# antekone/libarchive

Measured on AMD Instinct MI355X. Metric: decompressed MiB/s (whole node), lz4 filter, XXH32 verified, bit-exact, higher is better.
Workload: dtype u8; 1 GPU; C2: raw-format + lz4 filter, 16.00 GiB decoded per GPU, 262144 independent 64 KiB blocks per GPU in frames of 16, block+content+header XXH32 verified; compressed_bytes_per_gpu=7527480016, decoded_bytes_per_gpu=17179869184, unique_region_mib=1024, tiles=16, collectives=RCCL (nccl backend), expand_kernel=auto

## Files before the change

include/la_gpu.h:

```cpp
#ifndef LA_GPU_H
#define LA_GPU_H

#include <stddef.h>
#include <stdint.h>

#ifdef __cplusplus
extern "C" {
#endif

#define LA_GPU_ABI_VERSION 3

typedef enum la_rc {
	LA_OK            = 0,
	LA_ERR_NO_DEVICE = -1,
	LA_ERR_HIP       = -2,
	LA_ERR_ARG       = -3,
	LA_ERR_NOMEM     = -4
} la_rc;

typedef struct la_gpu_ctx la_gpu_ctx;

int         la_gpu_abi_version(void);
int         la_gpu_device_count(void);
int         la_gpu_open(int device, la_gpu_ctx **out);
// ... 141 lines not shown
	la_batch_summary   *d_summary;
	uint32_t            options;
	uint32_t            hist_len;
	const void         *d_carry_in;
	void               *d_carry_out;
} la_lz4_batch;
#define LA_XXH_CARRY_BYTES 64u

uint64_t la_gpu_lz4_workspace_bytes(uint32_t n_blocks, uint64_t src_bytes);

int la_gpu_lz4_decode(la_gpu_ctx *ctx, const la_lz4_batch *batch);

int la_gpu_lz4_debug_deps(la_gpu_ctx *ctx, const la_lz4_batch *batch, uint32_t block, uint64_t *seq_out,
    uint32_t *deps_out, uint32_t cap);

typedef struct la_gz_member {
	uint64_t src_off;
	uint32_t src_len;
	uint32_t dst_cap;
	uint64_t dst_off;
} la_gz_member;

typedef struct la_gz_result {
	uint32_t status;
	uint32_t out_len;
	uint32_t consumed;
	uint32_t crc32;
} la_gz_result;

typedef struct la_gz_batch {
// ... 378 lines not shown
```

libarchive_amd/_native.py:

```python
import ctypes as C
import os

import numpy as np

_PKG = os.path.dirname(os.path.abspath(__file__))
GPU_LIB_PATH = os.environ.get("LA_GPU_LIB") or os.path.join(_PKG, "csrc", "libla_gpu.so")
HOST_LIB_PATH = os.path.join(_PKG, "host", "libla_host.so")

LA_OK = 0

LZ4_BLOCK_DTYPE = np.dtype([("src_off", "<u8"), ("src_len", "<u4"), ("dst_cap", "<u4"),
                            ("flags", "<u4"), ("block_sum", "<u4")])
LZ4_FRAME_DTYPE = np.dtype([("desc_off", "<u8"), ("desc_len", "<u4"), ("first_block", "<u4"),
                            ("n_blocks", "<u4"), ("flags", "<u4"), ("content_sum", "<u4"),
                            ("reserved", "<u4")])
HASH_JOB_DTYPE = np.dtype([("off", "<u8"), ("len", "<u4"), ("seed", "<u4")])
SUMMARY_DTYPE = np.dtype([("total_out", "<u8"), ("n_bad_units", "<u4"), ("n_bad_frames", "<u4"),
                          ("first_bad_unit", "<u4"), ("first_bad_frame", "<u4"),
                          ("first_zero_unit", "<u4"), ("reserved", "<u4")])
GZ_MEMBER_DTYPE = np.dtype([("src_off", "<u8"), ("src_len", "<u4"), ("dst_cap", "<u4"), ("dst_off", "<u8")])
GZ_RESULT_DTYPE = np.dtype([("status", "<u4"), ("out_len", "<u4"), ("consumed", "<u4"), ("crc32", "<u4")])
assert LZ4_BLOCK_DTYPE.itemsize == 24 and LZ4_FRAME_DTYPE.itemsize == 32
assert HASH_JOB_DTYPE.itemsize == 16 and SUMMARY_DTYPE.itemsize == 32

# ... 218 lines not shown
        lib.la_gpu_sync.argtypes = [C.c_void_p]
        lib.la_gpu_last_error.argtypes = [C.c_void_p]
        lib.la_gpu_last_error.restype = C.c_char_p
        lib.la_gpu_reserve.argtypes = [C.c_void_p, C.c_uint64]
        lib.la_gpu_timer_start.argtypes = [C.c_void_p]
        lib.la_gpu_timer_stop.argtypes = [C.c_void_p, C.POINTER(C.c_float)]
        lib.la_gpu_profile_enable.argtypes = [C.c_void_p, C.c_int]
        lib.la_gpu_profile_read.argtypes = [C.c_void_p, C.POINTER(C.c_float), C.POINTER(C.c_char_p), C.c_int]
        lib.la_gpu_xxh32_many.argtypes = [C.c_void_p, C.c_void_p, C.c_void_p, C.c_uint32, C.c_void_p]
        lib.la_gpu_crc32_many.argtypes = [C.c_void_p, C.c_void_p, C.c_void_p, C.c_uint32, C.c_void_p]
        lib.la_gpu_lz4_workspace_bytes.argtypes = [C.c_uint32, C.c_uint64]
        lib.la_gpu_lz4_workspace_bytes.restype = C.c_uint64
        lib.la_gpu_lz4_decode.argtypes = [C.c_void_p, C.POINTER(_Lz4BatchC)]
        lib.la_gpu_lz4_debug_deps.argtypes = [C.c_void_p, C.POINTER(_Lz4BatchC), C.c_uint32, C.c_void_p, C.c_void_p,
                                              C.c_uint32]
        lib.la_gpu_lz4_compress.argtypes = [C.c_void_p, C.POINTER(_Lz4cBatchC)]
        lib.la_gpu_gzip_compress.argtypes = [C.c_void_p, C.POINTER(_GzcBatchC)]
        lib.la_gpu_gzip_compress_bound.restype = C.c_uint64
        lib.la_gpu_gzip_compress_bound.argtypes = [C.c_uint64, C.c_uint32]
        lib.la_gpu_gzip_compress_workspace_bytes.restype = C.c_uint64
        lib.la_gpu_gzip_compress_workspace_bytes.argtypes = [C.c_uint64, C.c_uint32]
        lib.la_gpu_lz4_compress_bound.restype = C.c_uint64
        lib.la_gpu_lz4_compress_bound.argtypes = [C.c_uint64, C.c_uint32, C.c_uint32]
        lib.la_gpu_lz4_compress_workspace_bytes.restype = C.c_uint64
        lib.la_gpu_lz4_compress_workspace_bytes.argtypes = [C.c_uint64, C.c_uint32, C.c_uint32]
        lib.la_gpu_gzip_decode.argtypes = [C.c_void_p, C.POINTER(_GzBatchC)]
        lib.la_gpu_zip_compress.argtypes = [C.c_void_p, C.POINTER(_ZipcBatchC)]
        lib.la_gpu_zip_compress_bound.restype = C.c_uint64
        lib.la_gpu_zip_compress_bound.argtypes = [C.c_uint64, C.c_uint32, C.c_uint32, C.c_uint64]
        lib.la_gpu_zip_compress_workspace_bytes.restype = C.c_uint64
# ... 221 lines not shown
        self._check(gpu_lib().la_gpu_xxh32_many(self._h, d_base_ptr, d_jobs_ptr, n, d_out_ptr), "la_gpu_xxh32_many")

    def crc32_many(self, d_base_ptr, d_jobs_ptr, n, d_out_ptr):
        self._check(gpu_lib().la_gpu_crc32_many(self._h, d_base_ptr, d_jobs_ptr, n, d_out_ptr), "la_gpu_crc32_many")

    def lz4_decode(self, batch: _Lz4BatchC):
        self._check(gpu_lib().la_gpu_lz4_decode(self._h, C.byref(batch)), "la_gpu_lz4_decode")

    def lz4_debug_deps(self, batch: _Lz4BatchC, block: int, cap: int = 4096):
        seq, deps = np.zeros(cap, dtype=np.uint64), np.zeros(cap, dtype=np.uint32)
        n = gpu_lib().la_gpu_lz4_debug_deps(self._h, C.byref(batch), block, seq.ctypes.data, deps.ctypes.data, cap)
        if n < 0:
            self._check(n, "la_gpu_lz4_debug_deps")
        return seq[:min(n, cap)], deps[:min(n, cap)]

    def lz4_compress(self, batch: _Lz4cBatchC):
        self._check(gpu_lib().la_gpu_lz4_compress(self._h, C.byref(batch)), "la_gpu_lz4_compress")

    def zstd_compress(self, batch: _ZstdcBatchC):
        self._check(gpu_lib().la_gpu_zstd_compress(self._h, C.byref(batch)), "la_gpu_zstd_compress")

    def bzip2_compress(self, batch: _Bz2cBatchC):
        self._check(gpu_lib().la_gpu_bzip2_compress(self._h, C.byref(batch)), "la_gpu_bzip2_compress")

    def gzip_compress(self, batch: _GzcBatchC):
        self._check(gpu_lib().la_gpu_gzip_compress(self._h, C.byref(batch)), "la_gpu_gzip_compress")

    def zip_compress(self, batch: _ZipcBatchC) -> int:
        rc = gpu_lib().la_gpu_zip_compress(self._h, C.byref(batch))
        if rc != LA_ERR_ARG:
# ... 38 lines not shown
```

libarchive_amd/csrc/la_api.hip:

```cpp
#include "la_dev.h"
#include <stdio.h>
#include <stdlib.h>
#include <string.h>
#include <new>

#define LA_MAX_SLICES 8
#define LA_GZ_LANES_MIN 8192u
#define LA_PROF_MAX_RANGES 64

struct la_gpu_ctx {
	int device;
	hipStream_t own_stream;
	hipStream_t stream;
	hipEvent_t ev0, ev1;
	hipEvent_t mark;
	void *ws;
	uint64_t ws_bytes;
	uint32_t *lz4_deps;
	uint64_t lz4_deps_cap;
	hipStream_t aux_stream;
	hipEvent_t slice_ev[LA_MAX_SLICES + 1];
	int prof_on;
	int prof_n;
	hipEvent_t prof_a[LA_PROF_MAX_RANGES], prof_b[LA_PROF_MAX_RANGES];
	const char *prof_name[LA_PROF_MAX_RANGES];
	char err[256];
};

static void prof_begin(la_gpu_ctx *c) { c->prof_n = 0; }
static int prof_open(la_gpu_ctx *c, const char *name, hipStream_t s)
{
	if (!c->prof_on || c->prof_n >= LA_PROF_MAX_RANGES)
		return -1;
	int h = c->prof_n++;
// ... 65 lines not shown
	for (int i = 0; i <= LA_MAX_SLICES; i++)
		(void)hipEventCreateWithFlags(&c->slice_ev[i], hipEventDisableTiming);
	c->stream = c->own_stream;
	*out = c;
	return LA_OK;
}

void la_gpu_close(la_gpu_ctx *c)
{
	if (!c)
		return;
	(void)hipSetDevice(c->device);
	(void)hipStreamSynchronize(c->stream);
	if (c->ws) (void)hipFree(c->ws);
	if (c->lz4_deps) (void)hipFree(c->lz4_deps);
	(void)hipEventDestroy(c->ev0);
	(void)hipEventDestroy(c->ev1);
	(void)hipEventDestroy(c->mark);
	for (int i = 0; i < LA_PROF_MAX_RANGES; i++) {
		(void)hipEventDestroy(c->prof_a[i]);
		(void)hipEventDestroy(c->prof_b[i]);
	}
	for (int i = 0; i <= LA_MAX_SLICES; i++)
		(void)hipEventDestroy(c->slice_ev[i]);
	(void)hipStreamSynchronize(c->aux_stream);
	(void)hipStreamDestroy(c->aux_stream);
	(void)hipStreamDestroy(c->own_stream);
	delete c;
}

// ... 185 lines not shown

uint64_t la_gpu_lz4_workspace_bytes(uint32_t n_blocks, uint64_t src_bytes)
{
	lz4_ws w;
	lz4_ws_carve(&w, NULL, n_blocks, src_bytes, true);
	return w.total;
}

static int lz4_deps_reserve(la_gpu_ctx *c, uint64_t words)
{
	if (words <= c->lz4_deps_cap)
		return LA_OK;
	HIPCHK(c, hipSetDevice(c->device));
	HIPCHK(c, hipStreamSynchronize(c->stream));
	HIPCHK(c, hipStreamSynchronize(c->aux_stream));
	if (c->lz4_deps) { HIPCHK(c, hipFree(c->lz4_deps)); c->lz4_deps = NULL; c->lz4_deps_cap = 0; }
	words = (words + 0x3FFFFull) & ~0x3FFFFull;
	HIPCHK(c, hipMalloc((void **)&c->lz4_deps, words * sizeof(uint32_t)));
	c->lz4_deps_cap = words;
	return LA_OK;
}

static bool lz4_uses_deps(const la_lz4_batch *bt)
{
	return !(bt->options & (LA_LZ4_OPT_GENERAL_ONLY | LA_LZ4_OPT_SEARCH_IN_EXPAND)) && bt->n_blocks &&
	    ((bt->options & LA_LZ4_OPT_EXPAND_INORDER) == 0 || !la_lz4_expand_inorder_takes(bt->src_bytes));
}

int la_gpu_lz4_decode(la_gpu_ctx *c, const la_lz4_batch *bt)
{
	if (!c || !bt)
		return LA_ERR_ARG;
	if (!bt->d_dst_off || (bt->n_blocks && (!bt->d_src || !bt->d_blocks || !bt->d_dst || !bt->d_out_len ||
// ... 10 lines not shown
		int rc = la_gpu_reserve(c, w.total);
		if (rc != LA_OK) return rc;
	}
	lz4_ws_carve(&w, (uint8_t *)c->ws, bt->n_blocks, bt->src_bytes, fast);
	const bool with_deps = lz4_uses_deps(bt);
	if (with_deps) {
		int rc = lz4_deps_reserve(c, w.table_cap);
		if (rc != LA_OK) return rc;
	}
	hipStream_t sx = c->stream;
	hipStream_t sp = c->aux_stream;
	const uint32_t n = bt->n_blocks;
	const la_expand_job xj = {	 bt->d_src, bt->src_bytes, bt->d_blocks, n, bt->d_dst, bt->dst_cap, bt->d_dst_off,
	    bt->d_out_len, bt->d_block_status, w.nseq, fast ? w.table : NULL, w.table_off,
	    LA_LZ4_LONG_SEQ_BYTES,
	    with_deps ? c->lz4_deps : NULL };

	prof_begin(c);
	HIPCHK(c, hipEventRecord(c->slice_ev[LA_MAX_SLICES], sx));
	HIPCHK(c, hipStreamWaitEvent(sp, c->slice_ev[LA_MAX_SLICES], 0));

	if (n)
		HIPCHK(c, hipMemsetAsync(bt->d_block_status, 0, (size_t)n * sizeof(uint32_t), sp));
	if (fast) {
		la_launch_lz4_table_caps(sp, bt->d_blocks, n, w.caps);
		la_launch_scan_u32(sp, w.caps, n, w.table_off, w.scan);
	}
	if (verify && n)
		HIPCHK(c, hipMemsetAsync(w.sum_status, 0, (size_t)n * sizeof(uint32_t), sp));
	if (bt->options & LA_LZ4_OPT_PARSE_V1) {
		if (verify && n)
// ... 1 lines not shown
		prof_range(c, "lz4_parse", sp, [&] {
			la_launch_lz4_parse(sp, bt->d_src, bt->src_bytes, bt->d_blocks, n, bt->d_out_len, w.nseq,
			    bt->d_block_status, fast ? w.table : NULL, w.table_off, w.table_cap);
		});
	} else {
		prof_range(c, "lz4_parse", sp, [&] {
			la_launch_lz4_parse_staged(sp, bt->d_src, bt->src_bytes, bt->d_blocks, n, bt->d_out_len, w.nseq,
			    bt->d_block_status, verify ? w.sum_status : NULL, fast ? w.table : NULL, w.table_off, w.table_cap);
		});
	}
	HIPCHK(c, hipEventRecord(c->slice_ev[0], sp));

	HIPCHK(c, hipStreamWaitEvent(sx, c->slice_ev[0], 0));
	prof_range(c, "scan", sx, [&] { la_launch_scan_u32(sx, bt->d_out_len, n, bt->d_dst_off, w.scan); });
	if (with_deps)
		prof_range(c, "lz4_deps", sx, [&] { la_launch_lz4_deps(sx, xj, c->lz4_deps); });

	prof_range(c, fast ? "lz4_expand_general" : "lz4_expand", sx, [&] { la_launch_lz4_expand_general(sx, xj, bt->hist_len); });
	if (fast && poll)
		prof_range(c, "lz4_expand_big", sx, [&] { la_launch_lz4_expand_fast_big(sx, xj, w.big); });
	const uint32_t nsl = (fast && n >= 4u * 8192u) ? 4u : 1u;
	if (bt->n_frames && !verify)
		HIPCHK(c, hipMemsetAsync(bt->d_frame_status, 0, (size_t)bt->n_frames * sizeof(uint32_t), sx));
	for (uint32_t i = 0; i < nsl; i++) {
		const uint32_t first = (uint32_t)((uint64_t)n * i / nsl), last = (uint32_t)((uint64_t)n * (i + 1) / nsl);
		const la_expand_job sj = xj.slice(first, last - first);
		if (fast)
			prof_range(c, "lz4_expand", sx, [&] { (poll ? la_launch_lz4_expand_fast : la_launch_lz4_expand_inorder)(sx, sj); });
		if (bt->n_frames && verify) {
			HIPCHK(c, hipEventRecord(c->slice_ev[1 + i], sx));
			HIPCHK(c, hipStreamWaitEvent(sp, c->slice_ev[1 + i], 0));
// ... 31 lines not shown
	HIPCHK(c, hipMemcpyAsync(&ns, w.nseq + block, sizeof(ns), hipMemcpyDeviceToHost, c->stream));
	HIPCHK(c, hipMemcpyAsync(&toff, w.table_off + block, sizeof(toff), hipMemcpyDeviceToHost, c->stream));
	HIPCHK(c, hipStreamSynchronize(c->stream));
	if (ns == 0xFFFFFFFFu)
		return 0;
	if (ns > 0x7FFFFFFFu || toff > w.table_cap || ns > w.table_cap - toff)
		return LA_ERR_ARG;
	const uint32_t m = ns < cap ? ns : cap;
	if (m) {
		static_assert(sizeof(la_lz4_seq) == sizeof(uint64_t), "a table entry travels as one 64-bit value");
		HIPCHK(c, hipMemcpyAsync(seq_out, w.table + toff, (size_t)m * sizeof(uint64_t), hipMemcpyDeviceToHost, c->stream));
		HIPCHK(c, hipMemcpyAsync(deps_out, c->lz4_deps + toff, (size_t)m * sizeof(uint32_t), hipMemcpyDeviceToHost, c->stream));
		HIPCHK(c, hipStreamSynchronize(c->stream));
	}
	return (int)ns;
}

uint64_t la_gpu_zstd_workspace_bytes(uint32_t n_frames)
{
	return la_zstd_workspace_bytes(n_frames);
}

int la_gpu_zstd_decode(la_gpu_ctx *c, const la_zstd_batch *bt)
{
	if (!c || !bt)
		return LA_ERR_ARG;
	if (bt->n_frames && (!bt->d_src || !bt->d_frames || !bt->d_dst || !bt->d_results))
		return LA_ERR_ARG;
	const bool blocks = (bt->options & LA_ZSTD_OPT_BLOCK_PARALLEL) && bt->n_frames && bt->dst_cap <= 0xFFFFFFFFull;
	const uint64_t ws_frames = (la_zstd_workspace_bytes(bt->n_frames) + 255) & ~255ull;
// ... 551 lines not shown
```

libarchive_amd/csrc/la_dev.h:

```cpp
#ifndef LA_DEV_H
#define LA_DEV_H

#include <hip/hip_runtime.h>
#include <stdint.h>
#include "../../include/la_gpu.h"

#define LA_WAVE 64

__device__ __forceinline__ uint32_t ld_u32(const uint8_t *p)
{
	uint32_t v;
	__builtin_memcpy(&v, p, 4);
	return v;
}
__device__ __forceinline__ uint4 ld_u128(const uint8_t *p)
{
	uint4 v;
	__builtin_memcpy(&v, p, 16);
	return v;
}
__device__ __forceinline__ uint32_t rotl32(uint32_t x, int r)
{
	return __builtin_rotateleft32(x, r);
}
// ... 393 lines not shown
	const uint32_t s0 = mdst - off;
	if (mlen == 0 || s0 >= d)
		return false;
	const uint32_t span = mlen < off ? mlen : off;
	uint32_t hi = s0 + span - 1;
	if (hi >= d)
		hi = d - 1;
	*hi_byte = hi;
	return true;
}
__device__ __forceinline__ bool la_lz4_dep_drops_last(uint32_t hi_byte, uint32_t last_mstart)
{
	return hi_byte < last_mstart;
}

struct la_expand_job {
	const uint8_t *src;
	uint64_t src_bytes;
	const la_lz4_block *blocks;
	uint32_t n;
	uint8_t *dst;
	uint64_t dst_cap;
	const uint64_t *dst_off;
	const uint32_t *out_len;
	uint32_t *status;
	const uint32_t *nseq;
	const la_lz4_seq *table;
	const uint64_t *table_off;
	uint32_t long_thr;
	const uint32_t *deps;

	la_expand_job slice(uint32_t first, uint32_t count) const
	{
		return la_expand_job{ src, src_bytes, blocks + first, count, dst, dst_cap, dst_off + first, out_len + first,
		    status + first, nseq + first, table, table_off + first, long_thr, deps };
	}
};

void la_launch_lz4_table_caps(hipStream_t s, const la_lz4_block *d_blocks, uint32_t n, uint32_t *d_caps);
void la_launch_lz4_parse(hipStream_t s, const uint8_t *d_src, uint64_t src_bytes,
    const la_lz4_block *d_blocks, uint32_t n, uint32_t *d_out_len, uint32_t *d_nseq,
    uint32_t *d_status, la_lz4_seq *d_table , const uint64_t *d_table_off,
    uint64_t table_cap );
void la_launch_lz4_parse_staged(hipStream_t s, const uint8_t *d_src, uint64_t src_bytes,
    const la_lz4_block *d_blocks, uint32_t n, uint32_t *d_out_len, uint32_t *d_nseq,
    uint32_t *d_status, uint32_t *d_sum_status, la_lz4_seq *d_table, const uint64_t *d_table_off,
    uint64_t table_cap);
void la_launch_lz4_expand_general(hipStream_t s, const la_expand_job &j, uint32_t hist_len);
void la_launch_lz4_expand_fast(hipStream_t s, const la_expand_job &j);
void la_launch_lz4_expand_fast_big(hipStream_t s, const la_expand_job &j, uint32_t *d_big );
void la_launch_lz4_deps(hipStream_t s, const la_expand_job &j, uint32_t *d_deps);

bool la_lz4_expand_inorder_takes(uint64_t src_bytes);
void la_launch_lz4_expand_inorder(hipStream_t s, const la_expand_job &j);

uint64_t la_zstd_workspace_bytes(uint32_t n_frames);
void la_launch_zstd_frames(hipStream_t s, const uint8_t *d_src, uint64_t src_bytes, const la_zstd_frame *d_frames, uint32_t n,
    uint8_t *d_dst, uint64_t dst_cap, la_zstd_result *d_results, uint8_t *ws, uint32_t options,
    const uint32_t *d_only );
uint64_t la_zstd_blocks_workspace_bytes(uint32_t n_frames, uint64_t src_bytes, uint64_t dst_cap);
const uint32_t *la_zstd_blocks_todo(const uint8_t *ws);
void la_launch_zstd_blocks(hipStream_t s, const uint8_t *d_src, uint64_t src_bytes, const la_zstd_frame *d_frames, uint32_t n,
    uint8_t *d_dst, uint64_t dst_cap, la_zstd_result *d_results, uint8_t *ws, uint32_t options);

uint64_t la_bzip2_workspace_bytes(uint32_t n, uint32_t level);
uint32_t la_bzip2_max_blocks(uint32_t level);
// ... 135 lines not shown
```

libarchive_amd/csrc/la_lz4_deps.hip:

```cpp
#include "la_dev.h"

#define DEPS_THREADS 256
#define DEPS_SLOTS   (LA_LZ4_FAST_MAXSEQ / DEPS_THREADS)

__global__ __launch_bounds__(DEPS_THREADS) void lz4_deps_kernel(const la_lz4_block *__restrict__ blocks, uint32_t n,
    uint64_t dst_cap, const uint64_t *__restrict__ dst_off, const uint32_t *__restrict__ out_len,
    const uint32_t *__restrict__ status, const uint32_t *__restrict__ nseq, const la_lz4_seq *__restrict__ table,
    const uint64_t *__restrict__ table_off, uint32_t long_thr, uint32_t *__restrict__ deps)
{
	__shared__ uint16_t dstpos[LA_LZ4_FAST_MAXSEQ];
	__shared__ uint16_t mstart[LA_LZ4_FAST_MAXSEQ];
	__shared__ uint16_t cmap[2048];

	const uint32_t bi = blockIdx.x;
	if (bi >= n)
		return;
	const uint32_t olen = out_len[bi], ns = nseq[bi];
	if (la_lz4_route(blocks[bi], status[bi], olen, ns, dst_off[bi], dst_cap, true, long_thr) != LA_XR_WINDOW)
		return;
	const uint32_t tid = threadIdx.x;
	const uint64_t *const tab = (const uint64_t *)(const void *)(table + table_off[bi]);
	uint32_t *const out = deps + table_off[bi];

	uint64_t ent[DEPS_SLOTS];
#pragma unroll
	for (uint32_t r = 0; r < DEPS_SLOTS; r++) {
		const uint32_t k = r * DEPS_THREADS + tid;
		ent[r] = k < ns ? tab[k] : 0;
	}
#pragma unroll
	for (uint32_t r = 0; r < DEPS_SLOTS; r++) {
		if (r * DEPS_THREADS >= ns)
			break;
		const uint32_t k = r * DEPS_THREADS + tid;
		if (k < ns) {
			const uint32_t d = (uint32_t)(ent[r] >> 32) & 0xFFFFu;
			dstpos[k] = (uint16_t)d;
			mstart[k] = (uint16_t)(d + ((uint32_t)(ent[r] >> 16) & 0xFFFFu));
		}
	}
	__syncthreads();
#pragma unroll
	for (uint32_t r = 0; r < DEPS_SLOTS; r++) {
		if (r * DEPS_THREADS >= ns)
			break;
		const uint32_t k = r * DEPS_THREADS + tid;
		const uint32_t after = k + 1 < ns ? (uint32_t)dstpos[k + 1] : (olen & 0xFFFFu);
		ent[r] = (ent[r] & ~0xFFFFull) | after;
	}
#pragma unroll
	for (uint32_t r = 0; r < DEPS_SLOTS; r++) {
		if (r * DEPS_THREADS >= ns)
			break;
		const uint32_t k = r * DEPS_THREADS + tid;
		if (k < ns) {
			const uint32_t d = (uint32_t)(ent[r] >> 32) & 0xFFFFu;
			uint32_t nxt = (uint32_t)ent[r] & 0xFFFFu;
			if (nxt < d)
				nxt = 65536u;
			if (k == 0)
				for (uint32_t c = 0; (c << 5) < d; c++)
					cmap[c] = 0;
			for (uint32_t c = (d + 31) >> 5; (c << 5) < nxt; c++)
				cmap[c] = (uint16_t)k;
		}
	}
	__syncthreads();

#pragma unroll
	for (uint32_t r = 0; r < DEPS_SLOTS; r++) {
		if (r * DEPS_THREADS >= ns)
			break;
		const uint32_t k = r * DEPS_THREADS + tid;
		const uint64_t e = ent[r];
// ... 18 lines not shown
		while (q + 1 < kq && dstpos[q + 1] <= s0)
			q++;
		if (qe < q)
			qe = q;
		while (qe + 1 < ke && dstpos[qe + 1] <= hi)
			qe++;
		if (k < ns) {
			uint32_t cnt = 0;
			if (waits)
				cnt = qe - q + 1 - (la_lz4_dep_drops_last(hi, mstart[qe]) ? 1u : 0u);
			out[k] = q | (cnt << 16);
		}
	}
}

void la_launch_lz4_deps(hipStream_t s, const la_expand_job &j, uint32_t *d_deps)
{
	if (j.n == 0) return;
	hipLaunchKernelGGL(lz4_deps_kernel, dim3(j.n), dim3(DEPS_THREADS), 0, s, j.blocks, j.n, j.dst_cap, j.dst_off,
	    j.out_len, j.status, j.nseq, j.table, j.table_off, j.long_thr, d_deps);
}
```

libarchive_amd/csrc/la_lz4_fast.hip:

```cpp
#include "la_dev.h"

#ifndef POLL_SLEEP
#define POLL_SLEEP 1
#endif
#ifndef FAST_THREADS
#define FAST_THREADS 512
#endif
#ifndef LBATCH
#define LBATCH 2
#endif
#ifndef FAST_MIN_WAVES
#define FAST_MIN_WAVES 4
#endif
#define FAST_WAVES   (FAST_THREADS / 64)

#ifdef LA_DIAG
__device__ unsigned long long *la_diag_stamps;
#define STAMP(slot)                                                                       \
	do {                                                                              \
		if (threadIdx.x == 0 && la_diag_stamps)                                    \
			la_diag_stamps[(size_t)blockIdx.x * 8 + (slot)] = __builtin_readcyclecounter(); \
	} while (0)
#else
#define STAMP(slot) do { } while (0)
// ... 15 lines not shown
{
	return *(const uint64_t *)(const void *)(t + k);
}
#define SEQ_LIT_SRC(e) ((uint32_t)((e) & 0xFFFFu))
#define SEQ_LIT_LEN(e) ((uint32_t)(((e) >> 16) & 0xFFFFu))
#define SEQ_DST(e)     ((uint32_t)(((e) >> 32) & 0xFFFFu))
#define SEQ_OFF(e)     ((uint32_t)((e) >> 48))

template <uint32_t MAXSEQ, bool SEG, bool DEPS>
__global__ __launch_bounds__(FAST_THREADS, FAST_MIN_WAVES) void lz4_expand_fast_kernel(
    const uint8_t *__restrict__ src, uint64_t src_bytes, const la_lz4_block *__restrict__ blocks,
    uint32_t n, uint8_t *__restrict__ dst, uint64_t dst_cap, const uint64_t *__restrict__ dst_off,
    const uint32_t *__restrict__ out_len, uint32_t *status_out,
    const uint32_t *__restrict__ nseq, const la_lz4_seq *__restrict__ table,
    const uint64_t *__restrict__ table_off, const uint32_t *__restrict__ big_list,
    const uint32_t *__restrict__ big_count, uint32_t long_thr, const uint32_t *__restrict__ deps)
{
	static_assert(!(SEG && DEPS), "the dependency words number a block's sequences from its first one");
	const uint32_t *status = status_out;
	__shared__ __attribute__((aligned(16))) uint8_t win[16 + 65536 + 96];
	__shared__ uint16_t dstpos[MAXSEQ + 4];
	__shared__ uint32_t donebits[MAXSEQ / 32];
	__shared__ uint16_t chunk_first[2048 + 8];

	auto do_block = [&](const uint32_t bi) __attribute__((always_inline)) {
	if (bi >= n)
		return;
	const la_lz4_block b = blocks[bi];
	const uint32_t olen = out_len[bi];
	const uint32_t ns_all = nseq[bi];
	const uint64_t doff = dst_off[bi];
	static_assert(MAXSEQ == LA_LZ4_FAST_MAXSEQ, "la_lz4_route splits the window kernels' blocks at LA_LZ4_FAST_MAXSEQ");
	if (la_lz4_route(b, status[bi], olen, ns_all, doff, dst_cap, true, long_thr) != (SEG ? LA_XR_WINDOW_SEG : LA_XR_WINDOW))
		return;

	STAMP(0);
	const uint32_t tid = threadIdx.x, lane = tid & 63, wave = tid >> 6;
	const la_lz4_seq *const tab_all = table + table_off[bi];
// ... 10 lines not shown
		vv[u][0] = vv[u][1] = vv[u][2] = vv[u][3] = 0;
		if (c0 < b.src_len) {
			if ((uint64_t)c0 + 32 <= s_room) {
				const uint4 a = ld_u128(s + c0), bq = ld_u128(s + c0 + 16);
				vv[u][0] = ((uint64_t)a.y << 32) | a.x; vv[u][1] = ((uint64_t)a.w << 32) | a.z;
				vv[u][2] = ((uint64_t)bq.y << 32) | bq.x; vv[u][3] = ((uint64_t)bq.w << 32) | bq.z;
			} else {
				for (uint32_t i = 0; c0 + i < s_room && i < 32; i++) {
					const uint64_t by = (uint64_t)s[c0 + i] << (8 * (i & 7));
					if (i < 8) vv[u][0] |= by; else if (i < 16) vv[u][1] |= by;
					else if (i < 24) vv[u][2] |= by; else vv[u][3] |= by;
				}
			}
		}
	}
	auto segment = [&](const uint32_t kb) __attribute__((always_inline)) {
	const la_lz4_seq *const tab = tab_all + kb;
	const uint32_t ns = ns_all - kb < MAXSEQ ? ns_all - kb : MAXSEQ;
	uint32_t cb = 0, seg_prev_end = 0;
	if (kb) {
		const seq_t pvb = seq_load(tab_all, kb - 1);
		seg_prev_end = SEQ_LIT_SRC(pvb) + SEQ_LIT_LEN(pvb);
		cb = seg_prev_end >> 5;
	}
	seq_t ent[MAXSTEPS];
	uint32_t prev_end[MAXSTEPS];
	uint32_t dw[MAXSTEPS];
#pragma unroll
	for (uint32_t r = 0; r < MAXSTEPS; r++) {
		ent[r] = 0;
		prev_end[r] = 0;
		dw[r] = 0;
	}
#pragma unroll
	for (uint32_t r = 0; r < MAXSTEPS; r++) {
		if (r * FAST_THREADS >= ns)
			break;
		const uint32_t k = fast_seq_index(r, wave, lane);
		ent[r] = k < ns ? seq_load(tab, k) : 0;
		const seq_t pv = ((k > 0 || kb > 0) && k < ns) ? seq_load(tab_all, kb + k - 1) : 0;
		prev_end[r] = SEQ_LIT_SRC(pv) + SEQ_LIT_LEN(pv);
	}
	if (tid < MAXSEQ / 32)
		donebits[tid] = 0;
	if (tid == 0) {
		dstpos[ns] = kb + ns < ns_all ? (uint16_t)SEQ_DST(seq_load(tab_all, kb + ns)) : (uint16_t)olen;
		if ((cb << 5) < seg_prev_end)
			chunk_first[0] = 0;
	}
#pragma unroll
	for (uint32_t r = 0; r < MAXSTEPS; r++) {
		if (r * FAST_THREADS >= ns)
			break;
		const uint32_t k = fast_seq_index(r, wave, lane);
		if (k < ns) {
			const uint32_t le = SEQ_LIT_SRC(ent[r]) + SEQ_LIT_LEN(ent[r]);
			for (uint32_t c = (prev_end[r] + 31) >> 5; (c << 5) < le; c++)
				chunk_first[c - cb] = (uint16_t)k;
			dstpos[k] = (uint16_t)SEQ_DST(ent[r]);
			if (k + 1 == ns)
				chunk_first[2048] = (uint16_t)(((le + 31) >> 5) - cb);
		}
	}
	__syncthreads();
#ifdef LA_DIAG_L
	STAMP(6);
#endif

	const uint32_t nlit_chunks = chunk_first[2048];
	for (uint32_t base = 0; base < nlit_chunks; base += LBATCH * FAST_THREADS) {
		uint32_t kk[LBATCH];
		seq_t pe[LBATCH][6];
#pragma unroll
		for (int u = 0; u < LBATCH; u++) {
			const uint32_t c = base + u * FAST_THREADS + tid;
			kk[u] = c < nlit_chunks ? (uint32_t)chunk_first[c] : 0xFFFFFFFFu;
			if (base != 0 || kb != 0) {
				vv[u][0] = vv[u][1] = vv[u][2] = vv[u][3] = 0;
				const uint32_t c0 = (cb + c) << 5;
				if (c < nlit_chunks) {
					if ((uint64_t)c0 + 32 <= s_room) {
						const uint4 a = ld_u128(s + c0), bq = ld_u128(s + c0 + 16);
						vv[u][0] = ((uint64_t)a.y << 32) | a.x; vv[u][1] = ((uint64_t)a.w << 32) | a.z;
						vv[u][2] = ((uint64_t)bq.y << 32) | bq.x; vv[u][3] = ((uint64_t)bq.w << 32) | bq.z;
					} else {
						for (uint32_t i = 0; c0 + i < s_room && i < 32; i++) {
							const uint64_t by = (uint64_t)s[c0 + i] << (8 * (i & 7));
							if (i < 8) vv[u][0] |= by; else if (i < 16) vv[u][1] |= by;
							else if (i < 24) vv[u][2] |= by; else vv[u][3] |= by;
						}
					}
// ... 42 lines not shown
			bool fin = false;
#pragma unroll
			for (int t = 0; t < 6; t++)
				if (!fin)
					fin = (kk[u] + t >= ns) || put(pe[u][t], kb != 0 && kk[u] + t == 0);
			for (uint32_t k = kk[u] + 6; !fin && k < ns; k++)
				fin = put(seq_load(tab, k), false);
		}
	}
	if (DEPS) {
#pragma unroll
		for (uint32_t r = 0; r < MAXSTEPS; r++) {
			const uint32_t k = fast_seq_index(r, wave, lane);
			dw[r] = (r * FAST_THREADS < ns && k < ns) ? deps[table_off[bi] + k] : 0;
		}
	}
	STAMP(1);
	__syncthreads();
	STAMP(2);

	uint32_t qcur[MAXSTEPS];
	if constexpr (DEPS) {
#pragma unroll
		for (uint32_t r = 0; r < MAXSTEPS; r++)
			qcur[r] = dw[r];
#ifdef LA_DIAG_M
		STAMP(6);
#endif
	} else {
#ifndef FAST_BSEARCH
// ... 277 lines not shown
	if (la_lz4_route(blocks[i], status[i], out_len[i], nseq[i], 0, ~0ull, true, long_thr) == LA_XR_WINDOW_SEG)
		big_list[atomicAdd(big_count, 1u)] = i;
}

#ifdef LA_DIAG
extern "C" int la_diag_set_stamps(void *d_buf)
{
	unsigned long long *p = (unsigned long long *)d_buf;
	return (int)hipMemcpyToSymbol(HIP_SYMBOL(la_diag_stamps), &p, sizeof(p));
}
#endif

void la_launch_lz4_expand_fast(hipStream_t s, const la_expand_job &j)
{
	if (j.n == 0) return;
	if (j.deps)
		hipLaunchKernelGGL((lz4_expand_fast_kernel<LA_LZ4_FAST_MAXSEQ, false, true>), dim3(j.n), dim3(FAST_THREADS), 0, s,
		    j.src, j.src_bytes, j.blocks, j.n, j.dst, j.dst_cap, j.dst_off, j.out_len, j.status, j.nseq,
		    j.table, j.table_off, (const uint32_t *)nullptr, (const uint32_t *)nullptr, j.long_thr, j.deps);
	else
		hipLaunchKernelGGL((lz4_expand_fast_kernel<LA_LZ4_FAST_MAXSEQ, false, false>), dim3(j.n), dim3(FAST_THREADS), 0, s,
		    j.src, j.src_bytes, j.blocks, j.n, j.dst, j.dst_cap, j.dst_off, j.out_len, j.status, j.nseq,
		    j.table, j.table_off, (const uint32_t *)nullptr, (const uint32_t *)nullptr, j.long_thr, (const uint32_t *)nullptr);
}

void la_launch_lz4_expand_fast_big(hipStream_t s, const la_expand_job &j, uint32_t *d_big)
{
	if (j.n == 0) return;
	(void)hipMemsetAsync(d_big, 0, sizeof(uint32_t), s);
	hipLaunchKernelGGL(lz4_classify_kernel, dim3((j.n + 255) / 256), dim3(256), 0, s, j.blocks, j.n, j.status, j.nseq,
	    d_big + 1, d_big, j.out_len, j.long_thr);
	const uint32_t grid = j.n < 1024u ? j.n : 1024u;
	hipLaunchKernelGGL((lz4_expand_fast_kernel<LA_LZ4_FAST_MAXSEQ, true, false>), dim3(grid), dim3(FAST_THREADS), 0, s,
	    j.src, j.src_bytes, j.blocks, j.n, j.dst, j.dst_cap, j.dst_off, j.out_len, j.status, j.nseq,
	    j.table, j.table_off, (const uint32_t *)(d_big + 1), (const uint32_t *)d_big, j.long_thr, (const uint32_t *)nullptr);
}
```

Measured before the change: 653,300 MiB/s.

## Precompute literal chunk-to-sequence plan in deps kernel for fast LZ4 expand

The deps kernel now also writes a per-block literal plan that maps each 32-byte literal chunk to the sequence owning it. When deps are present, the fast expand kernel reads this plan from global memory instead of rebuilding chunk_first in shared memory. This removes the prev_end table loads and the shared chunk-map build from the expand kernel and shrinks its shared memory footprint. The cost is an extra device buffer, extra global writes in the deps kernel and extra global reads in expand.

```diff
diff --git a/include/la_gpu.h b/include/la_gpu.h
--- a/include/la_gpu.h
+++ b/include/la_gpu.h
@@ -179,6 +179,9 @@
 int la_gpu_lz4_debug_deps(la_gpu_ctx *ctx, const la_lz4_batch *batch, uint32_t block, uint64_t *seq_out,
     uint32_t *deps_out, uint32_t cap);
 
+int la_gpu_lz4_debug_literal_plan(la_gpu_ctx *ctx, const la_lz4_batch *batch, uint32_t block, uint16_t *plan_out,
+    uint32_t cap);
+
 typedef struct la_gz_member {
 	uint64_t src_off;
 	uint32_t src_len;
diff --git a/libarchive_amd/_native.py b/libarchive_amd/_native.py
--- a/libarchive_amd/_native.py
+++ b/libarchive_amd/_native.py
@@ -256,6 +256,7 @@
         lib.la_gpu_lz4_decode.argtypes = [C.c_void_p, C.POINTER(_Lz4BatchC)]
         lib.la_gpu_lz4_debug_deps.argtypes = [C.c_void_p, C.POINTER(_Lz4BatchC), C.c_uint32, C.c_void_p, C.c_void_p,
                                               C.c_uint32]
+        lib.la_gpu_lz4_debug_literal_plan.argtypes = [C.c_void_p, C.POINTER(_Lz4BatchC), C.c_uint32, C.c_void_p, C.c_uint32]
         lib.la_gpu_lz4_compress.argtypes = [C.c_void_p, C.POINTER(_Lz4cBatchC)]
         lib.la_gpu_gzip_compress.argtypes = [C.c_void_p, C.POINTER(_GzcBatchC)]
         lib.la_gpu_gzip_compress_bound.restype = C.c_uint64
@@ -507,6 +508,13 @@
             self._check(n, "la_gpu_lz4_debug_deps")
         return seq[:min(n, cap)], deps[:min(n, cap)]
 
+    def lz4_debug_literal_plan(self, batch: _Lz4BatchC, block: int, cap: int = 2049):
+        plan = np.zeros(cap, dtype=np.uint16)
+        n = gpu_lib().la_gpu_lz4_debug_literal_plan(self._h, C.byref(batch), block, plan.ctypes.data, cap)
+        if n < 0:
+            self._check(n, "la_gpu_lz4_debug_literal_plan")
+        return plan[:min(n, cap)]
+
     def lz4_compress(self, batch: _Lz4cBatchC):
         self._check(gpu_lib().la_gpu_lz4_compress(self._h, C.byref(batch)), "la_gpu_lz4_compress")
 
diff --git a/libarchive_amd/csrc/la_api.hip b/libarchive_amd/csrc/la_api.hip
--- a/libarchive_amd/csrc/la_api.hip
+++ b/libarchive_amd/csrc/la_api.hip
@@ -18,6 +18,7 @@
 	uint64_t ws_bytes;
 	uint32_t *lz4_deps;
 	uint64_t lz4_deps_cap;
+	uint8_t *lz4_plan;
 	hipStream_t aux_stream;
 	hipEvent_t slice_ev[LA_MAX_SLICES + 1];
 	int prof_on;
@@ -113,6 +114,7 @@
 	(void)hipStreamSynchronize(c->stream);
 	if (c->ws) (void)hipFree(c->ws);
 	if (c->lz4_deps) (void)hipFree(c->lz4_deps);
+	if (c->lz4_plan) (void)hipFree(c->lz4_plan);
 	(void)hipEventDestroy(c->ev0);
 	(void)hipEventDestroy(c->ev1);
 	(void)hipEventDestroy(c->mark);
@@ -328,9 +330,12 @@
 	HIPCHK(c, hipSetDevice(c->device));
 	HIPCHK(c, hipStreamSynchronize(c->stream));
 	HIPCHK(c, hipStreamSynchronize(c->aux_stream));
-	if (c->lz4_deps) { HIPCHK(c, hipFree(c->lz4_deps)); c->lz4_deps = NULL; c->lz4_deps_cap = 0; }
+	c->lz4_deps_cap = 0;
+	if (c->lz4_deps) { HIPCHK(c, hipFree(c->lz4_deps)); c->lz4_deps = NULL; }
+	if (c->lz4_plan) { HIPCHK(c, hipFree(c->lz4_plan)); c->lz4_plan = NULL; }
 	words = (words + 0x3FFFFull) & ~0x3FFFFull;
 	HIPCHK(c, hipMalloc((void **)&c->lz4_deps, words * sizeof(uint32_t)));
+	HIPCHK(c, hipMalloc((void **)&c->lz4_plan, words));
 	c->lz4_deps_cap = words;
 	return LA_OK;
 }
@@ -371,7 +376,7 @@
 	const la_expand_job xj = {	 bt->d_src, bt->src_bytes, bt->d_blocks, n, bt->d_dst, bt->dst_cap, bt->d_dst_off,
 	    bt->d_out_len, bt->d_block_status, w.nseq, fast ? w.table : NULL, w.table_off,
 	    LA_LZ4_LONG_SEQ_BYTES,
-	    with_deps ? c->lz4_deps : NULL };
+	    with_deps ? c->lz4_deps : NULL, with_deps ? c->lz4_plan : NULL };
 
 	prof_begin(c);
 	HIPCHK(c, hipEventRecord(c->slice_ev[LA_MAX_SLICES], sx));
@@ -403,7 +408,7 @@
 	HIPCHK(c, hipStreamWaitEvent(sx, c->slice_ev[0], 0));
 	prof_range(c, "scan", sx, [&] { la_launch_scan_u32(sx, bt->d_out_len, n, bt->d_dst_off, w.scan); });
 	if (with_deps)
-		prof_range(c, "lz4_deps", sx, [&] { la_launch_lz4_deps(sx, xj, c->lz4_deps); });
+		prof_range(c, "lz4_deps", sx, [&] { la_launch_lz4_deps(sx, xj, c->lz4_deps, c->lz4_plan); });
 
 	prof_range(c, fast ? "lz4_expand_general" : "lz4_expand", sx, [&] { la_launch_lz4_expand_general(sx, xj, bt->hist_len); });
 	if (fast && poll)
@@ -465,6 +470,37 @@
 		HIPCHK(c, hipStreamSynchronize(c->stream));
 	}
 	return (int)ns;
+}
+
+int la_gpu_lz4_debug_literal_plan(la_gpu_ctx *c, const la_lz4_batch *bt, uint32_t block, uint16_t *plan_out, uint32_t cap)
+{
+	if (!c || !bt || block >= bt->n_blocks || (cap && !plan_out) || !lz4_uses_deps(bt))
+		return LA_ERR_ARG;
+	lz4_ws w;
+	lz4_ws_carve(&w, (uint8_t *)c->ws, bt->n_blocks, bt->src_bytes, true);
+	if (!c->ws || w.total > c->ws_bytes || w.table_cap > c->lz4_deps_cap || !c->lz4_plan)
+		return LA_ERR_ARG;
+	la_lz4_block b;
+	uint32_t ns = 0, st = 0, olen = 0;
+	uint64_t toff[2] = { 0, 0 }, doff = 0;
+	HIPCHK(c, hipMemcpyAsync(&b, bt->d_blocks + block, sizeof(b), hipMemcpyDeviceToHost, c->stream));
+	HIPCHK(c, hipMemcpyAsync(&ns, w.nseq + block, sizeof(ns), hipMemcpyDeviceToHost, c->stream));
+	HIPCHK(c, hipMemcpyAsync(&st, bt->d_block_status + block, sizeof(st), hipMemcpyDeviceToHost, c->stream));
+	HIPCHK(c, hipMemcpyAsync(&olen, bt->d_out_len + block, sizeof(olen), hipMemcpyDeviceToHost, c->stream));
+	HIPCHK(c, hipMemcpyAsync(&doff, bt->d_dst_off + block, sizeof(doff), hipMemcpyDeviceToHost, c->stream));
+	HIPCHK(c, hipMemcpyAsync(toff, w.table_off + block, sizeof(toff), hipMemcpyDeviceToHost, c->stream));
+	HIPCHK(c, hipStreamSynchronize(c->stream));
+	if (la_lz4_route(b, st, olen, ns, doff, bt->dst_cap, true, LA_LZ4_LONG_SEQ_BYTES) != LA_XR_WINDOW)
+		return 0;
+	const uint32_t m = la_lz4_plan_entries(b.src_len);
+	if (toff[0] > toff[1] || toff[1] > w.table_cap || 2ull * m > toff[1] - toff[0])
+		return LA_ERR_ARG;
+	const uint32_t take = m < cap ? m : cap;
+	if (take) {
+		HIPCHK(c, hipMemcpyAsync(plan_out, c->lz4_plan + toff[0], (size_t)take * sizeof(uint16_t), hipMemcpyDeviceToHost, c->stream));
+		HIPCHK(c, hipStreamSynchronize(c->stream));
+	}
+	return (int)m;
 }
 
 uint64_t la_gpu_zstd_workspace_bytes(uint32_t n_frames)
diff --git a/libarchive_amd/csrc/la_dev.h b/libarchive_amd/csrc/la_dev.h
--- a/libarchive_amd/csrc/la_dev.h
+++ b/libarchive_amd/csrc/la_dev.h
@@ -431,6 +431,16 @@
 	return hi_byte < last_mstart;
 }
 
+#define LA_LZ4_PLAN_NONE 0xFFFFu
+__host__ __device__ __forceinline__ uint32_t la_lz4_lit_chunk_edge(uint32_t lit_end)
+{
+	return (lit_end + 31u) >> 5;
+}
+__host__ __device__ __forceinline__ uint32_t la_lz4_plan_entries(uint32_t src_len)
+{
+	return la_lz4_lit_chunk_edge(src_len) + 1u;
+}
+
 struct la_expand_job {
 	const uint8_t *src;
 	uint64_t src_bytes;
@@ -446,11 +456,12 @@
 	const uint64_t *table_off;
 	uint32_t long_thr;
 	const uint32_t *deps;
+	const uint8_t *lit_plan;
 
 	la_expand_job slice(uint32_t first, uint32_t count) const
 	{
 		return la_expand_job{ src, src_bytes, blocks + first, count, dst, dst_cap, dst_off + first, out_len + first,
-		    status + first, nseq + first, table, table_off + first, long_thr, deps };
+		    status + first, nseq + first, table, table_off + first, long_thr, deps, lit_plan };
 	}
 };
 
@@ -466,7 +477,7 @@
 void la_launch_lz4_expand_general(hipStream_t s, const la_expand_job &j, uint32_t hist_len);
 void la_launch_lz4_expand_fast(hipStream_t s, const la_expand_job &j);
 void la_launch_lz4_expand_fast_big(hipStream_t s, const la_expand_job &j, uint32_t *d_big );
-void la_launch_lz4_deps(hipStream_t s, const la_expand_job &j, uint32_t *d_deps);
+void la_launch_lz4_deps(hipStream_t s, const la_expand_job &j, uint32_t *d_deps, uint8_t *d_plan);
 
 bool la_lz4_expand_inorder_takes(uint64_t src_bytes);
 void la_launch_lz4_expand_inorder(hipStream_t s, const la_expand_job &j);
diff --git a/libarchive_amd/csrc/la_lz4_deps.hip b/libarchive_amd/csrc/la_lz4_deps.hip
--- a/libarchive_amd/csrc/la_lz4_deps.hip
+++ b/libarchive_amd/csrc/la_lz4_deps.hip
@@ -6,7 +6,7 @@
 __global__ __launch_bounds__(DEPS_THREADS) void lz4_deps_kernel(const la_lz4_block *__restrict__ blocks, uint32_t n,
     uint64_t dst_cap, const uint64_t *__restrict__ dst_off, const uint32_t *__restrict__ out_len,
     const uint32_t *__restrict__ status, const uint32_t *__restrict__ nseq, const la_lz4_seq *__restrict__ table,
-    const uint64_t *__restrict__ table_off, uint32_t long_thr, uint32_t *__restrict__ deps)
+    const uint64_t *__restrict__ table_off, uint32_t long_thr, uint32_t *__restrict__ deps, uint8_t *__restrict__ lit_plan)
 {
 	__shared__ uint16_t dstpos[LA_LZ4_FAST_MAXSEQ];
 	__shared__ uint16_t mstart[LA_LZ4_FAST_MAXSEQ];
@@ -21,6 +21,8 @@
 	const uint32_t tid = threadIdx.x;
 	const uint64_t *const tab = (const uint64_t *)(const void *)(table + table_off[bi]);
 	uint32_t *const out = deps + table_off[bi];
+	uint16_t *const plan = (uint16_t *)(void *)(lit_plan + table_off[bi]);
+	const uint32_t nchunks = la_lz4_lit_chunk_edge(blocks[bi].src_len);
 
 	uint64_t ent[DEPS_SLOTS];
 #pragma unroll
@@ -34,9 +36,8 @@
 			break;
 		const uint32_t k = r * DEPS_THREADS + tid;
 		if (k < ns) {
-			const uint32_t d = (uint32_t)(ent[r] >> 32) & 0xFFFFu;
-			dstpos[k] = (uint16_t)d;
-			mstart[k] = (uint16_t)(d + ((uint32_t)(ent[r] >> 16) & 0xFFFFu));
+			dstpos[k] = (uint16_t)((uint32_t)(ent[r] >> 32) & 0xFFFFu);
+			mstart[k] = (uint16_t)(((uint32_t)ent[r] & 0xFFFFu) + ((uint32_t)(ent[r] >> 16) & 0xFFFFu));
 		}
 	}
 	__syncthreads();
@@ -45,9 +46,30 @@
 		if (r * DEPS_THREADS >= ns)
 			break;
 		const uint32_t k = r * DEPS_THREADS + tid;
+		if (k < ns) {
+			const uint32_t le = ((uint32_t)ent[r] & 0xFFFFu) + ((uint32_t)(ent[r] >> 16) & 0xFFFFu);
+			const uint32_t pe = k ? (uint32_t)mstart[k - 1] : 0u;
+			uint32_t cend = la_lz4_lit_chunk_edge(le);
+			if (cend > nchunks)
+				cend = nchunks;
+			for (uint32_t c = la_lz4_lit_chunk_edge(pe); c < cend; c++)
+				plan[c] = (uint16_t)k;
+			if (k + 1 == ns) {
+				for (uint32_t c = cend; c < nchunks; c++)
+					plan[c] = (uint16_t)LA_LZ4_PLAN_NONE;
+				plan[nchunks] = (uint16_t)cend;
+			}
+		}
+	}
+#pragma unroll
+	for (uint32_t r = 0; r < DEPS_SLOTS; r++) {
+		if (r * DEPS_THREADS >= ns)
+			break;
+		const uint32_t k = r * DEPS_THREADS + tid;
 		const uint32_t after = k + 1 < ns ? (uint32_t)dstpos[k + 1] : (olen & 0xFFFFu);
 		ent[r] = (ent[r] & ~0xFFFFull) | after;
 	}
+	__syncthreads();
 #pragma unroll
 	for (uint32_t r = 0; r < DEPS_SLOTS; r++) {
 		if (r * DEPS_THREADS >= ns)
@@ -58,6 +80,7 @@
 			uint32_t nxt = (uint32_t)ent[r] & 0xFFFFu;
 			if (nxt < d)
 				nxt = 65536u;
+			mstart[k] = (uint16_t)(d + ((uint32_t)(ent[r] >> 16) & 0xFFFFu));
 			if (k == 0)
 				for (uint32_t c = 0; (c << 5) < d; c++)
 					cmap[c] = 0;
@@ -106,9 +129,9 @@
 	}
 }
 
-void la_launch_lz4_deps(hipStream_t s, const la_expand_job &j, uint32_t *d_deps)
+void la_launch_lz4_deps(hipStream_t s, const la_expand_job &j, uint32_t *d_deps, uint8_t *d_plan)
 {
 	if (j.n == 0) return;
 	hipLaunchKernelGGL(lz4_deps_kernel, dim3(j.n), dim3(DEPS_THREADS), 0, s, j.blocks, j.n, j.dst_cap, j.dst_off,
-	    j.out_len, j.status, j.nseq, j.table, j.table_off, j.long_thr, d_deps);
+	    j.out_len, j.status, j.nseq, j.table, j.table_off, j.long_thr, d_deps, d_plan);
 }
diff --git a/libarchive_amd/csrc/la_lz4_fast.hip b/libarchive_amd/csrc/la_lz4_fast.hip
--- a/libarchive_amd/csrc/la_lz4_fast.hip
+++ b/libarchive_amd/csrc/la_lz4_fast.hip
@@ -53,14 +53,15 @@
     const uint32_t *__restrict__ out_len, uint32_t *status_out,
     const uint32_t *__restrict__ nseq, const la_lz4_seq *__restrict__ table,
     const uint64_t *__restrict__ table_off, const uint32_t *__restrict__ big_list,
-    const uint32_t *__restrict__ big_count, uint32_t long_thr, const uint32_t *__restrict__ deps)
+    const uint32_t *__restrict__ big_count, uint32_t long_thr, const uint32_t *__restrict__ deps,
+    const uint8_t *__restrict__ lit_plan)
 {
 	static_assert(!(SEG && DEPS), "the dependency words number a block's sequences from its first one");
 	const uint32_t *status = status_out;
 	__shared__ __attribute__((aligned(16))) uint8_t win[16 + 65536 + 96];
 	__shared__ uint16_t dstpos[MAXSEQ + 4];
 	__shared__ uint32_t donebits[MAXSEQ / 32];
-	__shared__ uint16_t chunk_first[2048 + 8];
+	__shared__ uint16_t chunk_first[DEPS ? 8 : 2048 + 8];
 
 	auto do_block = [&](const uint32_t bi) __attribute__((always_inline)) {
 	if (bi >= n)
@@ -101,6 +102,18 @@
 			}
 		}
 	}
+	const uint16_t *const plan = DEPS ? (const uint16_t *)(const void *)(lit_plan + table_off[bi]) : nullptr;
+	const uint32_t plan_chunks = la_lz4_lit_chunk_edge(b.src_len);
+	uint32_t kk0[LBATCH];
+#pragma unroll
+	for (int u = 0; u < LBATCH; u++) {
+		kk0[u] = LA_LZ4_PLAN_NONE;
+		if constexpr (DEPS) {
+			const uint32_t c = u * FAST_THREADS + tid;
+			if (c < plan_chunks)
+				kk0[u] = plan[c];
+		}
+	}
 	auto segment = [&](const uint32_t kb) __attribute__((always_inline)) {
 	const la_lz4_seq *const tab = tab_all + kb;
 	const uint32_t ns = ns_all - kb < MAXSEQ ? ns_all - kb : MAXSEQ;
@@ -125,43 +138,63 @@
 			break;
 		const uint32_t k = fast_seq_index(r, wave, lane);
 		ent[r] = k < ns ? seq_load(tab, k) : 0;
-		const seq_t pv = ((k > 0 || kb > 0) && k < ns) ? seq_load(tab_all, kb + k - 1) : 0;
-		prev_end[r] = SEQ_LIT_SRC(pv) + SEQ_LIT_LEN(pv);
-	}
-	if (tid < MAXSEQ / 32)
-		donebits[tid] = 0;
-	if (tid == 0) {
-		dstpos[ns] = kb + ns < ns_all ? (uint16_t)SEQ_DST(seq_load(tab_all, kb + ns)) : (uint16_t)olen;
-		if ((cb << 5) < seg_prev_end)
+		if constexpr (!DEPS) {
+			const seq_t pv = ((k > 0 || kb > 0) && k < ns) ? seq_load(tab_all, kb + k - 1) : 0;
+			prev_end[r] = SEQ_LIT_SRC(pv) + SEQ_LIT_LEN(pv);
+		}
+	}
+	auto publish = [&]() __attribute__((always_inline)) {
+		if (tid < MAXSEQ / 32)
+			donebits[tid] = 0;
+		if (tid == 0)
+			dstpos[ns] = kb + ns < ns_all ? (uint16_t)SEQ_DST(seq_load(tab_all, kb + ns)) : (uint16_t)olen;
+#pragma unroll
+		for (uint32_t r = 0; r < MAXSTEPS; r++) {
+			if (r * FAST_THREADS >= ns)
+				break;
+			const uint32_t k = fast_seq_index(r, wave, lane);
+			if (k < ns)
+				dstpos[k] = (uint16_t)SEQ_DST(ent[r]);
+		}
+	};
+	if constexpr (!DEPS) {
+		publish();
+		if (tid == 0 && (cb << 5) < seg_prev_end)
 			chunk_first[0] = 0;
-	}
-#pragma unroll
-	for (uint32_t r = 0; r < MAXSTEPS; r++) {
-		if (r * FAST_THREADS >= ns)
-			break;
-		const uint32_t k = fast_seq_index(r, wave, lane);
-		if (k < ns) {
-			const uint32_t le = SEQ_LIT_SRC(ent[r]) + SEQ_LIT_LEN(ent[r]);
-			for (uint32_t c = (prev_end[r] + 31) >> 5; (c << 5) < le; c++)
-				chunk_first[c - cb] = (uint16_t)k;
-			dstpos[k] = (uint16_t)SEQ_DST(ent[r]);
-			if (k + 1 == ns)
-				chunk_first[2048] = (uint16_t)(((le + 31) >> 5) - cb);
-		}
-	}
-	__syncthreads();
+#pragma unroll
+		for (uint32_t r = 0; r < MAXSTEPS; r++) {
+			if (r * FAST_THREADS >= ns)
+				break;
+			const uint32_t k = fast_seq_index(r, wave, lane);
+			if (k < ns) {
+				const uint32_t le = SEQ_LIT_SRC(ent[r]) + SEQ_LIT_LEN(ent[r]);
+				for (uint32_t c = la_lz4_lit_chunk_edge(prev_end[r]); c < la_lz4_lit_chunk_edge(le); c++)
+					chunk_first[c - cb] = (uint16_t)k;
+				if (k + 1 == ns)
+					chunk_first[2048] = (uint16_t)(la_lz4_lit_chunk_edge(le) - cb);
+			}
+		}
+		__syncthreads();
+	}
 #ifdef LA_DIAG_L
 	STAMP(6);
 #endif
 
-	const uint32_t nlit_chunks = chunk_first[2048];
+	uint32_t nlit_chunks = plan_chunks;
+	if constexpr (!DEPS)
+		nlit_chunks = chunk_first[2048];
 	for (uint32_t base = 0; base < nlit_chunks; base += LBATCH * FAST_THREADS) {
 		uint32_t kk[LBATCH];
 		seq_t pe[LBATCH][6];
 #pragma unroll
 		for (int u = 0; u < LBATCH; u++) {
 			const uint32_t c = base + u * FAST_THREADS + tid;
-			kk[u] = c < nlit_chunks ? (uint32_t)chunk_first[c] : 0xFFFFFFFFu;
+			if constexpr (DEPS) {
+				const uint32_t e = base == 0 ? kk0[u] : c < nlit_chunks ? (uint32_t)plan[c] : (uint32_t)LA_LZ4_PLAN_NONE;
+				kk[u] = e == LA_LZ4_PLAN_NONE ? 0xFFFFFFFFu : e;
+			} else {
+				kk[u] = c < nlit_chunks ? (uint32_t)chunk_first[c] : 0xFFFFFFFFu;
+			}
 			if (base != 0 || kb != 0) {
 				vv[u][0] = vv[u][1] = vv[u][2] = vv[u][3] = 0;
 				const uint32_t c0 = (cb + c) << 5;
@@ -234,6 +267,7 @@
 			const uint32_t k = fast_seq_index(r, wave, lane);
 			dw[r] = (r * FAST_THREADS < ns && k < ns) ? deps[table_off[bi] + k] : 0;
 		}
+		publish();
 	}
 	STAMP(1);
 	__syncthreads();
@@ -541,14 +575,15 @@
 void la_launch_lz4_expand_fast(hipStream_t s, const la_expand_job &j)
 {
 	if (j.n == 0) return;
-	if (j.deps)
+	if (j.deps && j.lit_plan)
 		hipLaunchKernelGGL((lz4_expand_fast_kernel<LA_LZ4_FAST_MAXSEQ, false, true>), dim3(j.n), dim3(FAST_THREADS), 0, s,
 		    j.src, j.src_bytes, j.blocks, j.n, j.dst, j.dst_cap, j.dst_off, j.out_len, j.status, j.nseq,
-		    j.table, j.table_off, (const uint32_t *)nullptr, (const uint32_t *)nullptr, j.long_thr, j.deps);
+		    j.table, j.table_off, (const uint32_t *)nullptr, (const uint32_t *)nullptr, j.long_thr, j.deps, j.lit_plan);
 	else
 		hipLaunchKernelGGL((lz4_expand_fast_kernel<LA_LZ4_FAST_MAXSEQ, false, false>), dim3(j.n), dim3(FAST_THREADS), 0, s,
 		    j.src, j.src_bytes, j.blocks, j.n, j.dst, j.dst_cap, j.dst_off, j.out_len, j.status, j.nseq,
-		    j.table, j.table_off, (const uint32_t *)nullptr, (const uint32_t *)nullptr, j.long_thr, (const uint32_t *)nullptr);
+		    j.table, j.table_off, (const uint32_t *)nullptr, (const uint32_t *)nullptr, j.long_thr, (const uint32_t *)nullptr,
+		    (const uint8_t *)nullptr);
 }
 
 void la_launch_lz4_expand_fast_big(hipStream_t s, const la_expand_job &j, uint32_t *d_big)
@@ -560,5 +595,6 @@
 	const uint32_t grid = j.n < 1024u ? j.n : 1024u;
 	hipLaunchKernelGGL((lz4_expand_fast_kernel<LA_LZ4_FAST_MAXSEQ, true, false>), dim3(grid), dim3(FAST_THREADS), 0, s,
 	    j.src, j.src_bytes, j.blocks, j.n, j.dst, j.dst_cap, j.dst_off, j.out_len, j.status, j.nseq,
-	    j.table, j.table_off, (const uint32_t *)(d_big + 1), (const uint32_t *)d_big, j.long_thr, (const uint32_t *)nullptr);
+	    j.table, j.table_off, (const uint32_t *)(d_big + 1), (const uint32_t *)d_big, j.long_thr, (const uint32_t *)nullptr,
+	    (const uint8_t *)nullptr);
 }
```

Result: faster. 667,200 MiB/s, median of 6 (+2.1%).
